# thodson-usgs/discontinuum

Measured on AMD Instinct MI355X. Metric: GP fits/sec (NLL+grad step) at n=8192 d=3, 1/2/4/8 MI355X, higher is better.
Workload: dtype f64

## Files before the change

### discontinuum_amd/_lib.py

```python
from __future__ import annotations

import ctypes as C
import os

_HERE = os.path.dirname(os.path.abspath(__file__))
LIB_PATH = os.path.join(_HERE, "libdgp_hip.so")

F64, F32 = 0, 1
MODEL_LOADEST, MODEL_RATING = 0, 1
OUT_NLL, OUT_QUAD, OUT_LOGDET, OUT_INFO, OUT_DTHETA, OUT_SUM_DR, OUT_DR_W0, OUT_SUM_DNOISE, OUT_LEN = 0, 1, 2, 3, 4, 28, 29, 31, 32
BUF_XT, BUF_A, BUF_T, BUF_S, BUF_Z, BUF_ALPHA = range(6)
BUF_SCAL = 7
OPT_LAUUM64_MAX_TILES, OPT_SYRK_SLOTS, OPT_TRTRI_SMALL, OPT_REFINE, OPT_SYRK_ORDER, OPT_LAUUM_ORDER, OPT_CHAIN_YIELD, OPT_FUSED_GRAD, OPT_GROUP_GEMM = range(9)
OPT_POTRF_SCHEDULE, OPT_POTRF_SWEEP, OPT_POTRF_SOLVE, OPT_POTRF_OVERLAP, OPT_POTRF_SLOTS, OPT_POTRF_TAIL, OPT_POTRF_TAIL_SWEEP = range(9, 16)
TIME_GRAM, TIME_POTRF, TIME_SYRK_SUM, TIME_SYRK_N, TIME_TRTRI, TIME_LAUUM, TIME_SOLVE, TIME_GRAD, TIME_SYRK_FLOP, TIME_COUNT = range(10)


class DGPLibraryError(RuntimeError):
    pass


class DGPError(RuntimeError):
    def __init__(self, code, where, msg):
        super().__init__(f"{where} failed with code {code}: {msg}")
        self.code = code


_vp, _i, _i64, _sz = C.c_void_p, C.c_int, C.c_int64, C.c_size_t
_dp = C.POINTER(C.c_double)

SIGNATURES = {
    "dgp_version": (_i, []),
    "dgp_last_error": (C.c_char_p, []),
    "dgp_model_ntheta": (_i, [_i, _i]),
    "dgp_composite_define": (_i, [C.POINTER(_i), _i, C.POINTER(_i)]),
    "dgp_padded_n": (_i64, [_i64]),
    "dgp_plan_create": (_i, [_i, _i, _i64, _i, C.POINTER(_vp)]),
# ... 93 lines not shown
```

### discontinuum_amd/csrc/dgp_api.hip

```cpp
#include <mutex>
#include <new>
#include <stdio.h>
#include <stdlib.h>
#include <string.h>
#include <utility>
#include <vector>

#include "../../include/dgp_hip.h"
#include "dgp_common.h"
#include "dgp_internal.h"

using namespace dgp;

static thread_local char g_err[256] = "";
static int fail(int code, const char* msg) {
  snprintf(g_err, sizeof(g_err), "%s", msg);
  return code;
}
static int hipfail(hipError_t e, const char* where) {
  snprintf(g_err, sizeof(g_err), "%s: %s", where, hipGetErrorString(e));
  return (int)e;
}

struct PinnedRing {
// ... 30 lines not shown
      if (have_ev[i]) (void)hipEventDestroy(ev[i]);
      if (buf[i]) (void)hipHostFree(buf[i]);
    }
  }
};

struct dgp_plan {
  int model, dtype, d, ntheta;
  PinnedRing ring;
  int* nsite_host;
  int B;
  size_t site_bytes;
  void* pre;
  void* pre2;
  int pre_ready;
  Tuning tune;
  int refine;
  int* nsite;
  const void* dr_w;
  int64_t n, N;
  size_t elem;
  char* ws;
  size_t ws_bytes;
  void *Xt, *A, *Tm, *S, *z, *alpha, *gpart, *spart, *scal, *snap;
  int* info;
  hipStream_t sc;
  int lookahead, early;
  int have_inputs, have_factor, have_inverse;
  hipStream_t s2, s3;
  hipEvent_t xev[8];
  int have_xev;
  hipEvent_t* ev;
  int nev;
  int timing, n_syrk, timed_valid;
  double syrk_flop;
  hipEvent_t* tev;
  hipEvent_t* sev;
  int nsev;
};
enum { TS_GRAM = 0, TS_POTRF, TS_TRTRI, TS_LAUUM, TS_SOLVE, TS_GRAD, TS_COUNT };

static size_t align_up(size_t x) { return (x + 255) & ~(size_t)255; }

struct Layout {
  size_t Xt, A, Tm, S, z, alpha, gpart, spart, scal, info, snap, total;
};
static Layout layout(const dgp_plan* p) {
  Layout L;
  const size_t e = p->elem, N = (size_t)p->N;
  size_t o = 0;
  L.Xt = o; o += align_up(e * N * p->d);
  L.A = o; o += align_up(e * N * N);
  L.Tm = o; o += align_up(e * N * N);
  L.S = o; o += align_up(e * N * N);
  L.z = o; o += align_up(e * N);
  L.alpha = o; o += align_up(e * N);
  L.gpart = o; o += align_up(e * (size_t)gram_grad_partials(p->N));
  L.spart = o; o += align_up(e * (size_t)solve_partials(p->N));
  L.scal = o; o += align_up(e * 16);
  L.info = o; o += align_up(sizeof(int) * POTRF_INFO_INTS);
  L.snap = o; o += align_up(e * 2 * DGP_TILE_HOST * DGP_TILE_HOST);
  L.total = o;
  return L;
}

static int default_lookahead() { return 2; }
static int group_size(int lookahead, int batch, long nbk) {
  if (!lookahead) return 0;
  if (const char* e = getenv("DGP_GROUP")) return atoi(e) < 2 ? 2 : atoi(e);
  if (batch >= 4) return 4;
  return nbk >= 256 ? 8 : (nbk >= 96 ? 4 : 2);
}

static int early_wg_cap() {
  const char* e = getenv("DGP_EARLY_WG_CAP");
  return e ? atoi(e) : 384;
}
#define EARLY_WG_CAP early_wg_cap()
static int early_reserved_cus() {
  const char* e = getenv("DGP_EARLY_RESERVED_CUS");
  const int v = e ? atoi(e) : 64;
  return v < 0 ? 0 : (v > 128 ? 128 : v);
}
#define EARLY_RESERVED_CUS early_reserved_cus()
// ... 98 lines not shown
  return 0;
}

int dgp_plan_set_workspace(dgp_plan* p, void* dev_ptr, size_t bytes) {
  if (!p || !dev_ptr) return fail(DGP_E_ARG, "dgp_plan_set_workspace: null");
  const Layout L = layout(p);
  if (bytes < dgp_plan_workspace_bytes(p))
    return fail(DGP_E_WORKSPACE, "dgp_plan_set_workspace: workspace too small");
  p->site_bytes = L.total;
  if (((uintptr_t)dev_ptr & 255) != 0) return fail(DGP_E_ARG, "dgp_plan_set_workspace: pointer must be 256-byte aligned");
  p->ws = (char*)dev_ptr;
  p->ws_bytes = bytes;
  p->Xt = p->ws + L.Xt;
  p->A = p->ws + L.A;
  p->Tm = p->ws + L.Tm;
  p->S = p->ws + L.S;
  p->z = p->ws + L.z;
  p->alpha = p->ws + L.alpha;
  p->gpart = p->ws + L.gpart;
  p->spart = p->ws + L.spart;
  p->scal = p->ws + L.scal;
  p->info = (int*)(p->ws + L.info);
  p->snap = p->ws + L.snap;
  p->pre = pre_scratch_bytes(p->B) ? (void*)(p->ws + L.total * (size_t)p->B) : nullptr;
  p->pre2 = p->pre ? (void*)((char*)p->pre + align_up(pre_scratch_bytes(p->B))) : nullptr;
  p->nsite = nullptr;
  p->dr_w = nullptr;
  if (p->B > 1) {
    p->nsite = (int*)(p->ws + L.total * (size_t)p->B + 2 * align_up(pre_scratch_bytes(p->B)));
    delete[] p->nsite_host;
    p->nsite_host = new (std::nothrow) int[(size_t)p->B];
    if (!p->nsite_host) return fail(DGP_E_ARG, "dgp_plan_set_workspace: out of host memory");
    for (int b = 0; b < p->B; ++b) p->nsite_host[b] = (int)p->n;
    hipError_t e = hipMemcpy(p->nsite, p->nsite_host, sizeof(int) * (size_t)p->B, hipMemcpyHostToDevice);
    if (e != hipSuccess) return hipfail(e, "dgp_plan_set_workspace: hipMemcpy");
  }
  p->have_inputs = p->have_factor = 0;
  return 0;
}

int dgp_plan_set_option(dgp_plan* p, int key, int64_t value) {
  if (!p) return fail(DGP_E_ARG, "dgp_plan_set_option: null plan");
  switch (key) {
    case DGP_OPT_LAUUM64_MAX_TILES:
      if (value < 0 || value > (1 << 30)) return fail(DGP_E_ARG, "dgp_plan_set_option: value out of range");
      p->tune.lauum64_max_tiles = (int)value;
// ... 19 lines not shown
      return 0;
    case DGP_OPT_GROUP_GEMM:
      p->tune.group_gemm = value ? 1 : 0;
      return 0;
    case DGP_OPT_POTRF_SCHEDULE:
      if (value < 0 || value > 1) return fail(DGP_E_ARG, "dgp_plan_set_option: value out of range");
      p->tune.potrf_schedule = (int)value;
      return 0;
    case DGP_OPT_POTRF_SWEEP:
    case DGP_OPT_POTRF_TAIL:
    case DGP_OPT_POTRF_TAIL_SWEEP:
      if (value < 0 || value > (1 << 20)) return fail(DGP_E_ARG, "dgp_plan_set_option: value out of range");
      (key == DGP_OPT_POTRF_SWEEP ? p->tune.potrf_sweep : key == DGP_OPT_POTRF_TAIL ? p->tune.potrf_tail : p->tune.potrf_tail_sweep) = (int)value;
      return 0;
    case DGP_OPT_POTRF_SOLVE:
      p->tune.potrf_solve = value ? 1 : 0;
      return 0;
    case DGP_OPT_POTRF_OVERLAP:
      p->tune.potrf_overlap = value ? 1 : 0;
      return 0;
    case DGP_OPT_POTRF_SLOTS:
      if (value < 1 || value > (1 << 20)) return fail(DGP_E_ARG, "dgp_plan_set_option: value out of range");
      p->tune.potrf_slots = (int)value;
      return 0;
    case DGP_OPT_REFINE:
      if (p->dtype != DGP_F32 && value) return fail(DGP_E_ARG, "dgp_plan_set_option: refinement applies to float32 plans");
      p->refine = value ? 1 : 0;
      return 0;
    default:
      return fail(DGP_E_ARG, "dgp_plan_set_option: unknown option");
  }
}
int dgp_plan_get_option(const dgp_plan* p, int key, int64_t* value) {
  if (!p || !value) return fail(DGP_E_ARG, "dgp_plan_get_option: null argument");
  switch (key) {
    case DGP_OPT_LAUUM64_MAX_TILES: *value = p->tune.lauum64_max_tiles; return 0;
    case DGP_OPT_SYRK_SLOTS: *value = p->tune.syrk_slots; return 0;
    case DGP_OPT_TRTRI_SMALL: *value = p->tune.trtri_small; return 0;
    case DGP_OPT_REFINE: *value = p->refine; return 0;
    case DGP_OPT_SYRK_ORDER: *value = p->tune.syrk_super; return 0;
    case DGP_OPT_LAUUM_ORDER: *value = p->tune.lauum_super; return 0;
    case DGP_OPT_CHAIN_YIELD: *value = p->tune.chain_yield; return 0;
    case DGP_OPT_FUSED_GRAD: *value = p->tune.fused_grad; return 0;
    case DGP_OPT_GROUP_GEMM: *value = p->tune.group_gemm; return 0;
    case DGP_OPT_POTRF_SCHEDULE:
      *value = p->tune.potrf_schedule < 0 ? (p->B >= 4 ? potrf_schedule_auto(p->B, p->N / DGP_TILE_HOST, p->elem) : 0) : p->tune.potrf_schedule;
      return 0;
    case DGP_OPT_POTRF_SWEEP: *value = p->tune.potrf_sweep; return 0;
    case DGP_OPT_POTRF_SOLVE: *value = p->tune.potrf_solve; return 0;
    case DGP_OPT_POTRF_OVERLAP: *value = p->tune.potrf_overlap; return 0;
    case DGP_OPT_POTRF_SLOTS: *value = p->tune.potrf_slots; return 0;
    case DGP_OPT_POTRF_TAIL: *value = p->tune.potrf_tail; return 0;
    case DGP_OPT_POTRF_TAIL_SWEEP: *value = p->tune.potrf_tail_sweep; return 0;
    default: return fail(DGP_E_ARG, "dgp_plan_get_option: unknown option");
  }
}

int dgp_plan_set_lookahead(dgp_plan* p, int level) {
  if (!p) return fail(DGP_E_ARG, "null plan");
  p->lookahead = level ? default_lookahead() : 0;
  p->early = level >= 2 && !getenv("DGP_NO_EARLY_TRTRI");
  return 0;
}

size_t dgp_plan_site_stride_bytes(const dgp_plan* p) { return p ? layout(p).total : 0; }

int dgp_plan_buffer(const dgp_plan* p, int which, void** dev_ptr, int64_t* ld) {
  if (!p || !dev_ptr || !p->ws) return fail(DGP_E_ARG, "dgp_plan_buffer: null / no workspace");
  void* q = nullptr;
  switch (which) {
    case DGP_BUF_XT: q = p->Xt; break;
    case DGP_BUF_A: q = p->A; break;
    case DGP_BUF_T: q = p->Tm; break;
    case DGP_BUF_S: q = p->S; break;
    case DGP_BUF_Z: q = p->z; break;
    case DGP_BUF_ALPHA: q = p->alpha; break;
// ... 273 lines not shown
  }
}

template <typename T>
static int run_grad(dgp_plan* p, const double* theta, void* dtheta, hipStream_t s) {
  return gram_grad<T>(p->model, p->d, (const T*)p->Xt, p->N, (int)p->n, theta, (const T*)p->S, (const T*)p->alpha,
                      (T*)p->gpart, (T*)dtheta, s, batch_of<T>(p), DGP_OUT_LEN, p->pre, p->pre_ready != 0);
}

template <typename T>
static int solve_overlap_mode(dgp_plan* p, hipStream_t s, hipStream_t* out) {
  static const int env = getenv("DGP_SOLVE_OVERLAP") ? atoi(getenv("DGP_SOLVE_OVERLAP")) : -1;
  const int mode = env >= 0 ? env : ((p->N >= 1024 && p->N <= 6144) ? 1 : 0);
  if (mode <= 0 || !p->lookahead || !p->ev || p->nev < 2) return 0;
  if (sizeof(T) == 4 && p->refine) return 0;
  if (mode == 1 && p->s2) {
    *out = p->s2;
    return 1;
  }
  StreamSet* st = stream_set(s);
  if (!st || make_stream(&st->rest, true)) return 0;
  *out = st->rest;
  return 2;
}

template <typename T>
static int fit_step(dgp_plan* p, const double* theta, const void* r, const void* noise, void* out, void* dr,
                    void* dnoise, int with_grad, hipStream_t s) {
  int rc;
  if ((rc = ensure_timing(p))) return rc;
  tick(p, TS_GRAM, 0, s);
  if ((rc = run_gram<T>(p, theta, noise, s))) return rc;
  tick(p, TS_GRAM, 1, s);
  if ((rc = ensure_async(p, s)) || (rc = ensure_early(p, s))) return rc;
  tick(p, TS_POTRF, 0, s);
  const int nbk = (int)(p->N / DGP_TILE_HOST);
  const bool early = early_applies(p) && p->s3 != nullptr;
  const Batch bt = batch_of<T>(p);
  if (early) {
    struct Early {
      dgp_plan* p;
      int ck[3];
      TrtriProgress st;
      int rc;
    } ctx{p, {nbk / 2, 3 * nbk / 4, 7 * nbk / 8}, {}, 0};
    if (const char* e = getenv("DGP_EARLY_CK")) {
// ... 17 lines not shown
      rc = potrf_split<T>((T*)p->A, p->N, (T*)p->Tm, (T*)p->scal, p->info, (T*)p->snap, s, p->sc, p->s2, p->ev,
                          p->timing ? p->sev : nullptr, &p->n_syrk, &p->syrk_flop, 3, ctx.ck, p->xev, on_ck, &ctx, split_start(p), group_size(p->lookahead, p->B, p->N / DGP_TILE_HOST), &p->tune);
    else
      rc = potrf<T>((T*)p->A, p->N, (T*)p->Tm, (T*)p->scal, p->info, group_size(p->lookahead, p->B, p->N / DGP_TILE_HOST), s, p->s2, p->ev,
                    p->timing ? p->sev : nullptr, &p->n_syrk, &p->syrk_flop, 3, ctx.ck, p->xev, on_ck, &ctx, bt);
    if (rc || (rc = ctx.rc)) return rc;
    tick(p, TS_POTRF, 1, s);
    tick(p, TS_TRTRI, 0, s);
    hipEventRecord(p->xev[3], s);
    hipStreamWaitEvent(p->s3, p->xev[3], 0);
    if ((rc = trtri_advance<T>((const T*)p->A, p->N, (T*)p->Tm, (T*)p->S, nbk, &ctx.st, p->s3, 0, nullptr, 0, 0, bt)))
      return rc;
    hipEventRecord(p->xev[4], p->s3);
    hipStreamWaitEvent(s, p->xev[4], 0);
    tick(p, TS_TRTRI, 1, s);
  } else {
    if ((rc = run_potrf<T>(p, s))) return rc;
    tick(p, TS_POTRF, 1, s);
    tick(p, TS_TRTRI, 0, s);
    if ((rc = run_trtri<T>(p, s))) return rc;
    tick(p, TS_TRTRI, 1, s);
  }
  const bool fused = with_grad && p->tune.fused_grad && lauum_grad_applies(p->model, p->N, bt);
  hipStream_t ss = s;
  const int ov = (with_grad && !fused) ? solve_overlap_mode<T>(p, s, &ss) : 0;
  if (ov) {
    hipEventRecord(p->ev[0], s);
    hipStreamWaitEvent(ss, p->ev[0], 0);
  }
  tick(p, TS_SOLVE, 0, ss);
  if ((rc = run_solve<T>(p, r, ss))) return rc;
  if ((rc = run_refine<T>(p, theta, r, noise, ss))) return rc;
  tick(p, TS_SOLVE, 1, ss);
  if (ov) hipEventRecord(p->ev[1], ss);
  p->timed_valid = 0;
  p->have_inverse = 0;
  if (!with_grad && ov) hipStreamWaitEvent(s, p->ev[1], 0);
  if (fused) {
    tick(p, TS_LAUUM, 0, s);
    void* staging = (p->pre && !p->pre_ready) ? p->ring.acquire(pre_scratch_bytes(p->B)) : nullptr;
    rc = lauum_grad<T>(p->model, p->d, (const T*)p->Tm, p->N, (T*)p->S, (const T*)p->Xt, (int)p->n, theta, (const T*)p->alpha,
                       (T*)p->gpart, (T*)out + DGP_OUT_DTHETA, s, bt, DGP_OUT_LEN, p->pre, p->pre_ready != 0, staging);
    if (staging) p->ring.commit(s);
    if (rc) return rc;
    p->pre_ready = 1;
    tick(p, TS_LAUUM, 1, s);
    tick(p, TS_GRAD, 0, s);
    tick(p, TS_GRAD, 1, s);
    p->timed_valid = p->timing && p->tev;
    p->have_inverse = 1;
  } else if (with_grad) {
    tick(p, TS_LAUUM, 0, s);
    if ((rc = run_lauum<T>(p, s))) return rc;
    tick(p, TS_LAUUM, 1, s);
    if (ov) hipStreamWaitEvent(s, p->ev[1], 0);
    tick(p, TS_GRAD, 0, s);
    if ((rc = run_grad<T>(p, theta, (T*)out + DGP_OUT_DTHETA, s))) return rc;
    tick(p, TS_GRAD, 1, s);
    p->timed_valid = p->timing && p->tev;
    p->have_inverse = 1;
  }
  const unsigned nwg = with_grad ? (unsigned)((p->n + 255) / 256) : 1u;
  finish_kernel<T><<<dim3(nwg, 1, (unsigned)bt.B), 256, 0, s>>>(
      (const T*)p->scal, p->info, (long)p->n, p->ntheta, !with_grad, (T*)out, bt.ws, bt.ws * (long)sizeof(T) / (long)sizeof(int), bt.ns,
      (const T*)p->alpha, (const T*)(with_grad ? p->dr_w : nullptr), (const T*)p->S, p->N, (T*)(with_grad ? dnoise : nullptr),
      (T*)(with_grad ? dr : nullptr), (T*)p->spart);
  p->have_factor = 1;
  return (int)hipGetLastError();
}

static size_t predict_site_bytes(const dgp_plan* p, int64_t m) {
  const size_t M = (size_t)round_up(m, DGP_TILE_HOST), e = p->elem;
  return align_up(e * M * p->d) + 2 * align_up(e * (size_t)p->N * M) + 3 * align_up(e * M) + align_up(e * 2 * PREDICT_SPLIT * M);
}
struct PreSlot {
  dgp_plan* p;
  void* staging;
  hipStream_t s;
  PreSlot(dgp_plan* plan, hipStream_t st) : p(plan), staging(plan->pre ? plan->ring.acquire(pre_scratch_bytes(plan->B)) : nullptr), s(st) {
    plan->pre_ready = 0;
  }
  ~PreSlot() {
    if (staging) p->ring.commit(s);
  }
};

template <typename T>
static int cross(dgp_plan* p, const double* theta, const void* Xs, int64_t m, void* work, void* Ks, hipStream_t s, long wbs = 0) {
  const long M = round_up(m, DGP_TILE_HOST);
  Batch wb;
  wb.B = p->B;
// ... 447 lines not shown
```

### discontinuum_amd/csrc/dgp_chol.hip

```cpp
#include <stdlib.h>
#include <string.h>
#include <algorithm>
#include <mutex>
#include "dgp_diag.h"
#include "dgp_gemm.h"
#include "dgp_gemm_dma.h"
#include "dgp_internal.h"
#include "dgp_schedule.h"

namespace dgp {

static constexpr int NB = DGP_TILE;
static constexpr int SMID_TABLE = 4096;
template <typename T>
struct Prefetch {
  static constexpr bool F64 = sizeof(T) == 8;
  static constexpr int LAUUM = F64 ? 2 : 4, TRTRI = F64 ? 1 : 4, SYRK = F64 ? 1 : 2;
};

#define DGP_INFO_CHAIN_TIMEOUT (-7)
#define CHAIN_WAIT_TICKS 200000000LL
__device__ __forceinline__ bool chain_reached(const int* word, int value) {
  return __hip_atomic_load(word, __ATOMIC_RELAXED, __HIP_MEMORY_SCOPE_AGENT) >= value;
}
// ... 105 lines not shown
    if (bi == bj && part == 1) return;
    syrk_tile<T, 64, 64, false, CMODE>(A, ld, k, nk, row0 + 64 * (part >> 1), col0 + 64 * (part & 1), smem);
  }
}

const Tuning& default_tuning() {
  static const Tuning t = [] {
    Tuning v;
    v.lauum64_max_tiles = getenv("DGP_LAUUM64") ? atoi(getenv("DGP_LAUUM64")) : 1000;
    v.syrk_slots = getenv("DGP_SYRK_SLOTS") ? atoi(getenv("DGP_SYRK_SLOTS")) : 512;
    v.trtri_small = getenv("DGP_TRTRI_SMALL") ? atol(getenv("DGP_TRTRI_SMALL")) : 1024;
    v.syrk_super = getenv("DGP_SYRK_ORDER") ? atoi(getenv("DGP_SYRK_ORDER")) : 0;
    v.lauum_super = getenv("DGP_LAUUM_ORDER") ? atoi(getenv("DGP_LAUUM_ORDER")) : 0;
    v.chain_yield = getenv("DGP_CHAIN_YIELD") ? atoi(getenv("DGP_CHAIN_YIELD")) : 1;
    v.fused_grad = getenv("DGP_FUSED_GRAD") ? atoi(getenv("DGP_FUSED_GRAD")) : 0;
    v.group_gemm = getenv("DGP_GROUP_GEMM") ? atoi(getenv("DGP_GROUP_GEMM")) : 0;
    v.potrf_schedule = getenv("DGP_POTRF_SCHEDULE") ? (atoi(getenv("DGP_POTRF_SCHEDULE")) != 0 ? 1 : 0) : -1;
    v.potrf_sweep = getenv("DGP_POTRF_SWEEP") ? std::max(0, atoi(getenv("DGP_POTRF_SWEEP"))) : 0;
    v.potrf_tail = getenv("DGP_POTRF_TAIL") ? std::max(0, atoi(getenv("DGP_POTRF_TAIL"))) : 0;
    v.potrf_tail_sweep = getenv("DGP_POTRF_TAIL_SWEEP") ? std::max(0, atoi(getenv("DGP_POTRF_TAIL_SWEEP"))) : 0;
    v.potrf_solve = getenv("DGP_POTRF_SOLVE") ? atoi(getenv("DGP_POTRF_SOLVE")) : 0;
    v.potrf_overlap = getenv("DGP_POTRF_OVERLAP") ? atoi(getenv("DGP_POTRF_OVERLAP")) : 0;
    v.potrf_slots = getenv("DGP_POTRF_SLOTS") ? std::max(1, atoi(getenv("DGP_POTRF_SLOTS"))) : 768;
    if (v.syrk_slots < 1) v.syrk_slots = 1;
    return v;
  }();
  return t;
}
int potrf_schedule_auto(int B, long nbk, int elem) { return (elem == 8 && B >= 32 && nbk > 4) ? 1 : 0; }
struct SyrkShape {
  int nfull, split;
  unsigned grid;
  explicit SyrkShape(int ntiles, int slots = 512) {
    if (slots < 1) slots = 1;
    const double cost[5] = {0, 1.0, 0.55, 0, 0.30};
    const int whole = ntiles / slots * slots, rem = ntiles - whole;
    nfull = ntiles;
    split = 1;
    double best = (ntiles + slots - 1) / slots * cost[1];
    for (int g = 2; g <= 4; g += 2) {
      const double c = whole / slots * cost[1] + (g * rem + slots - 1) / slots * cost[g];
      if (rem > 0 && c < best - 1e-9) {
        best = c;
        nfull = whole;
        split = g;
      }
// ... 808 lines not shown
    if (wcan > st->wdone[lvl]) st->wdone[lvl] = wcan;
    if (full > st->gdone[lvl]) st->gdone[lvl] = full;
  }
  if (early) st->pairs_used = nctr_pairs - el.pairs_left;
  return (int)hipGetLastError();
}

template <typename T>
static void trtri_group(const T* L, T* Tm, T* W, long N, int k0, int G, hipStream_t s, Batch bt) {
  for (int m = 1; m < G; m *= 2) {
    const int g0 = k0 / (2 * m), g1 = (k0 + G) / (2 * m);
    trtri_level<T, 0>(L, Tm, W, N, N, m, g0, g1, nullptr, s, bt);
    trtri_level<T, 1>(L, Tm, W, N, N, m, g0, g1, nullptr, s, bt);
  }
}

template <typename T>
int trtri(const T* L, const T* , long N, T* Tm, T* W, hipStream_t s, Batch bt,
          long ld) {
  TrtriProgress st;
  return trtri_advance<T>(L, N, Tm, W, (int)(N / NB), &st, s, 0, nullptr, 0, 0, bt, ld);
}

template <typename T>
__global__ __launch_bounds__(256, (TileCore<T, false, false>::OCC)) void lauum_kernel(const T* __restrict__ Tm, T* __restrict__ S, long ld,
                                                                                      int nbk, long bs, int super = 0) {
  Tm = site(Tm, bs);
  S = site(S, bs);
  using K = TileCore<T, false, false, 128, 128, Prefetch<T>::LAUUM, true, true>;
  using G = typename K::G;
  __shared__ T smem[K::SMEM_ELEMS];
  int bi, bj;
  if (super > 0) {
    const int x = (int)blockIdx.x & 7, j = (int)blockIdx.x >> 3, s2 = super * super;
    const int nsr = (nbk + super - 1) / super, st = (j / s2) * 8 + x;
    if (st >= nsr * (nsr + 1) / 2) return;
    int R, C;
    tri_decode(st, R, C);
    const int l = j % s2;
    bi = R * super + l / super;
    bj = C * super + l % super;
    if (bi >= nbk || bj > bi) return;
  } else {
    tri_decode(blockIdx.x, bi, bj);
  }
  typename G::acc_t acc[G::MI][G::NI];
  G::zero(acc);
  const T* base = Tm + (long)bi * NB * ld;
  T* out = S + (long)bi * NB * ld + (long)bj * NB;
  auto store = [&]() { K::foreach (acc, [&](int r, int c, T& v) { out[(long)r * ld + c] = v; }); };
  if (bi == bj) K::template run_tri<true, TRI_LOWER>(base + (long)bi * NB, ld, base + (long)bj * NB, ld, (nbk - bi) * (NB / 16), smem, acc, store);
  else K::template run_tri<true, TRI_ROW_LE>(base + (long)bi * NB, ld, base + (long)bj * NB, ld, (nbk - bi) * (NB / 16), smem, acc, store);
}

template <typename T>
__global__ __launch_bounds__(256, 2) void lauum64_kernel(const T* __restrict__ Tm, T* __restrict__ S, long ld, int nb64,
                                                         long bs) {
  Tm = site(Tm, bs);
  S = site(S, bs);
  using G = TileGemm<T, false, false, 64, 64>;
  __shared__ T smem[G::SMEM_ELEMS];
  int bi, bj;
  tri_decode(blockIdx.x, bi, bj);
  typename G::acc_t acc[G::MI][G::NI];
  G::zero(acc);
  const T* base = Tm + (long)bi * 64 * ld;
  G::template run<1, true>(base + (long)bi * 64, ld, base + (long)bj * 64, ld, (nb64 - bi) * (64 / 16), smem, acc);
  T* out = S + (long)bi * 64 * ld + (long)bj * 64;
  G::foreach (acc, [&](int r, int c, T& v) { out[(long)r * ld + c] = v; });
}

template <typename T>
int lauum(const T* Tm, long N, T* S, hipStream_t s, Batch bt) {
  const int nbk = (int)(N / NB);
  const int tiles = nbk * (nbk + 1) / 2;
  if ((long)tiles * bt.B <= bt.tuning().lauum64_max_tiles) {
    const int nb64 = 2 * nbk;
    lauum64_kernel<T><<<dim3((unsigned)(nb64 * (nb64 + 1) / 2), 1, (unsigned)bt.B), 256, 0, s>>>(Tm, S, N, nb64, bt.ws);
  } else {
    const int sup = bt.tuning().lauum_super;
    unsigned grid = (unsigned)tiles;
    if (sup > 0) {
      const int nsr = (nbk + sup - 1) / sup, nst = nsr * (nsr + 1) / 2;
      grid = (unsigned)((nst + 7) / 8 * 8 * sup * sup);
    }
    lauum_kernel<T><<<dim3(grid, 1, (unsigned)bt.B), 256, 0, s>>>(Tm, S, N, nbk, bt.ws, sup);
  }
  return (int)hipGetLastError();
}

template <typename T>
__global__ __launch_bounds__(256) void trmv_n_kernel(const T* __restrict__ Tm, long ld, const T* __restrict__ r, int n,
                                                     T* __restrict__ z, long bs, const int* __restrict__ ns, long rs) {
  Tm = site(Tm, bs);
  z = site(z, bs);
  r = site(r, rs);
  n = site_n(ns, n);
  const int lane = threadIdx.x & 63;
  const long i = (long)blockIdx.x * 4 + (threadIdx.x >> 6);
  const long jend = (i / NB + 1) * NB;
  const T* row = Tm + i * ld;
  T acc = T(0);
  for (long j = lane; j < jend; j += 64) acc += row[j] * (j < n ? r[j] : T(0));
  acc = wave_sum(acc);
  if (lane == 0) z[i] = acc;
}

#define DGP_TRMV_CHUNK 512
static inline int trmv_chunk(long N) { return N < 2048 ? 128 : DGP_TRMV_CHUNK; }
template <typename T>
// ... 297 lines not shown
  G::foreach (acc, [&](int r, int c, T& v) {
    const long q = (long)bq * NB + r, j = (long)bj * NB + c;
    if (q < ndraw && j < m) out[q * m + j] = v + (mean ? mean[j] : T(0));
  });
}

template <typename T>
int sample_draws(const T* L, long M, const T* Z, long Q, const T* mean, int m, int ndraw, T* out, hipStream_t s) {
  sample_draws_kernel<T><<<dim3((unsigned)(Q / NB), (unsigned)(M / NB)), 256, 0, s>>>(L, M, Z, Q, mean, m, ndraw, out);
  return (int)hipGetLastError();
}

#define DGP_INST(T)                                                                                              \
  template int posterior_cov<T>(const T*, long, long, T*, hipStream_t, int, long);                                          \
  template int sample_draws<T>(const T*, long, const T*, long, const T*, int, int, T*, hipStream_t);             \
  template int symv_lower<T>(const T*, long, const T*, int, const T*, T*, T*, T*, hipStream_t, Batch, long);     \
  template int potrf<T>(T*, long, T*, T*, int*, int, hipStream_t, hipStream_t, hipEvent_t*, hipEvent_t*, int*, double*, int, \
                        const int*, hipEvent_t*, void (*)(void*, int), void*, Batch, int, PotrfCarry*);                                                                                        \
  template int potrf_split<T>(T*, long, T*, T*, int*, T*, hipStream_t, hipStream_t, hipStream_t, hipEvent_t*, hipEvent_t*, int*, double*, \
                              int, const int*, hipEvent_t*, void (*)(void*, int), void*, int, int, const Tuning*);         \
  template int potrf_group<T>(T*, long, int, T*, T*, int*, int, int, hipStream_t);                                \
  template int trtri_advance<T>(const T*, long, T*, T*, int, TrtriProgress*, hipStream_t, int, int*, int, int, Batch, long);                   \
  template int trtri<T>(const T*, const T*, long, T*, T*, hipStream_t, Batch, long);                                        \
  template int lauum<T>(const T*, long, T*, hipStream_t, Batch);                                                      \
  template int solve<T>(const T*, long, const T*, int, T*, T*, T*, T*, hipStream_t, Batch);                           \
  template int refine_solve<T>(const T*, long, const T*, int, const double*, const T*, T*, T*, T*, T*, T*, hipStream_t, Batch, long, long); \
  template int finish<T>(const T*, const T*, long, int, T*, hipStream_t, Batch);                                      \
  template int predict_var<T>(const T*, long, const T*, long, T*, const T*, const T*, T*, T*, T*, hipStream_t, Batch, long);
DGP_INST(double)
DGP_INST(float)

}

#ifdef DGP_DIAG_LOG
extern "C" int dgp_debug_diag_log(unsigned long long* out_host) {
  return (int)hipMemcpyFromSymbol(out_host, HIP_SYMBOL(dgp::dgp_diag_log), sizeof(unsigned long long) * 4 * 1024);
}
#endif
```

### discontinuum_amd/csrc/dgp_internal.h

```cpp
#pragma once
#include <hip/hip_runtime.h>
#include <stdint.h>

#define DGP_TILE_HOST 128

namespace dgp {

inline long round_up(long n, long q) { return (n + q - 1) / q * q; }

#define DGP_MAX_BATCH_HOST 8
#define DGP_MAX_BATCH_SITES 1024
struct Tuning {
  int lauum64_max_tiles;
  int syrk_slots;
  long trtri_small;
  int syrk_super;
  int lauum_super;
  int chain_yield;
  int fused_grad;
  int group_gemm;
  int potrf_schedule;
  int potrf_sweep;
  int potrf_tail;
  int potrf_tail_sweep;
  int potrf_solve;
  int potrf_slots;
  int potrf_overlap;
};
const Tuning& default_tuning();
int potrf_schedule_auto(int B, long nbk, int elem);
struct Batch {
  int B = 1;
  long ws = 0;
  const int* ns = nullptr;
  const Tuning* tune = nullptr;
  void* W = nullptr;
  const Tuning& tuning() const { return tune ? *tune : default_tuning(); }
};
int model_ntheta(int model, int d);
int composite_define(const int* spec, int nspec);
bool composite_select(int model, int d);

template <typename T>
int pack_x(const T* X, int n, int d, long N, T* Xt, hipStream_t s, Batch bt = Batch());
template <typename T>
int gram_sym(int model, int d, const T* Xt, long N, int n, const double* theta, const T* noise, T* K, hipStream_t s,
             Batch bt = Batch(), void* pre_scratch = nullptr ,
             void* pre_staging = nullptr ,
             long k_stride = -1 , long noise_stride = -1 ,
             bool pre_ready = false );
// ... 44 lines not shown
                void* ck_ctx = nullptr, int k_start = 0 ,
                int G_old = 2 , const Tuning* tune = nullptr);
struct TrtriProgress {
  static constexpr int MAXLVL = 16;
  int wdone[MAXLVL] = {0}, gdone[MAXLVL] = {0};
  int pairs_used = 0;
};
template <typename T>
int trtri_advance(const T* L, long N, T* Tm, T* W, int ready_blocks, TrtriProgress* st, hipStream_t s, int wg_cap,
                  int* ctr , int nctr_pairs, int reserve_cus, Batch bt = Batch(),
                  long ld = 0 );
#define CHAIN_FLAG0 2
#define EARLY_CTR0 4
#define EARLY_CTR_PAIRS 125
#define POTRF_INFO_INTS (EARLY_CTR0 + 2 * EARLY_CTR_PAIRS + 4)
#define CHAIN_ABORT (POTRF_INFO_INTS - 4)
#define CHAIN_YIELD (POTRF_INFO_INTS - 3)
#define CHAIN_DIAG_DONE (POTRF_INFO_INTS - 2)
#define CHAIN_TICKET (POTRF_INFO_INTS - 1)
const unsigned char* reserved_cu_table(int nreserve, int* n_cu);
template <typename T>
int trtri(const T* L, const T* Dinv, long N, T* Tm, T* W, hipStream_t s, Batch bt = Batch(), long ld = 0);
template <typename T>
int lauum(const T* Tm, long N, T* S, hipStream_t s, Batch bt = Batch());
template <typename T>
int solve(const T* Tm, long N, const T* r, int n, T* z, T* alpha, T* partials, T* quad, hipStream_t s,
          Batch bt = Batch());
template <typename T>
int finish(const T* S, const T* alpha, long N, int n, T* dnoise, hipStream_t s, Batch bt = Batch());
template <typename T>
int refine_solve(const T* Tm, long N, const T* r, int n, const double* rho64, const T* rho32, T* z, T* delta, T* alpha,
                 T* partials, T* quad, hipStream_t s, Batch bt, long scratch_stride ,
                 long rho32_stride );
#define PREDICT_SPLIT 32
template <typename T>
int predict_var(const T* Tm, long N, const T* Ks, long M, T* V, const T* alpha, const T* kss, T* part, T* mean, T* var,
                hipStream_t s, Batch bt = Batch(), long wbs = 0);
long solve_partials(long N);
template <typename T>
int potrf_group(T* A, long ld, int nbk, T* Tinv, T* logdet, int* info, int k0, int W, hipStream_t s);
struct SlabMap {
  int W, world, rank;
  __host__ __device__ int gblock(int lb) const { return ((lb / W) * world + rank) * W + lb % W; }
};
template <typename T>
int gram_slab(int model, int d, const T* Xt, long N, int n, const double* theta, const T* noise, T* Aslab, long Cl,
              SlabMap sm, hipStream_t s);
// ... 29 lines not shown
```

### include/dgp_hip.h

```cpp
#ifndef DGP_HIP_H
#define DGP_HIP_H
#include <stddef.h>
#include <stdint.h>

#ifdef __cplusplus
extern "C" {
#endif

#define DGP_F64 0
#define DGP_F32 1
#define DGP_MODEL_LOADEST 0
#define DGP_MODEL_RATING 1

#define DGP_E_ARG (-1)
#define DGP_E_MODEL (-2)
#define DGP_E_WORKSPACE (-3)
#define DGP_E_STATE (-4)

#define DGP_OUT_NLL 0
#define DGP_OUT_QUAD 1
#define DGP_OUT_LOGDET 2
#define DGP_OUT_INFO 3
#define DGP_OUT_DTHETA 4
#define DGP_OUT_SUM_DR 28
// ... 23 lines not shown
size_t dgp_plan_workspace_bytes(const dgp_plan* plan);
int dgp_plan_set_batch(dgp_plan* plan, int batch);
int dgp_plan_batch(const dgp_plan* plan);
int dgp_plan_set_site_sizes(dgp_plan* plan, const int64_t* sizes_host, void* stream);
int dgp_plan_set_workspace(dgp_plan* plan, void* dev_ptr, size_t bytes);
int dgp_plan_set_dr_weights(dgp_plan* plan, const void* w_dev);
int dgp_plan_set_lookahead(dgp_plan* plan, int level);
#define DGP_OPT_LAUUM64_MAX_TILES 0
#define DGP_OPT_SYRK_SLOTS 1
#define DGP_OPT_TRTRI_SMALL 2
#define DGP_OPT_REFINE 3
#define DGP_OPT_SYRK_ORDER 4
#define DGP_OPT_LAUUM_ORDER 5
#define DGP_OPT_CHAIN_YIELD 6
#define DGP_OPT_FUSED_GRAD 7
#define DGP_OPT_GROUP_GEMM 8
#define DGP_OPT_POTRF_SCHEDULE 9
#define DGP_OPT_POTRF_SWEEP 10
#define DGP_OPT_POTRF_SOLVE 11
#define DGP_OPT_POTRF_OVERLAP 12
#define DGP_OPT_POTRF_SLOTS 13
#define DGP_OPT_POTRF_TAIL 14
#define DGP_OPT_POTRF_TAIL_SWEEP 15
int dgp_plan_set_option(dgp_plan* plan, int key, int64_t value);
int dgp_plan_get_option(const dgp_plan* plan, int key, int64_t* value_out);
int dgp_plan_buffer(const dgp_plan* plan, int which, void** dev_ptr, int64_t* ld);
size_t dgp_plan_site_stride_bytes(const dgp_plan* plan);

int dgp_set_inputs(dgp_plan* plan, const void* X_dev, void* stream);

int dgp_fit_step(dgp_plan* plan, const double* theta_host, const void* r_dev, const void* noise_dev,
                 void* out_dev, void* dr_dev, void* dnoise_dev, void* stream);

int dgp_factorize(dgp_plan* plan, const double* theta_host, const void* r_dev, const void* noise_dev,
                  void* out_dev, void* stream);

size_t dgp_predict_workspace_bytes(const dgp_plan* plan, int64_t m);
int dgp_predict(dgp_plan* plan, const double* theta_host, const void* Xs_dev, int64_t m, void* work_dev,
                size_t work_bytes, void* mean_dev, void* var_dev, void* stream);

int dgp_posterior_cov(dgp_plan* plan, const double* theta_host, const void* Xs_dev, int64_t m, void* work_dev,
                      size_t work_bytes, void* mean_dev, void* cov_dev, void* stream);

int dgp_sample_draws(int dtype, const void* L_dev, int64_t m, const void* Z_dev, int64_t ndraw, const void* mean_dev,
                     void* out_dev, void* stream);

// ... 83 lines not shown
```

Baseline: 118.0.

## Fuse alpha = S·r computation into LAUUM tile epilogue for f64

When the gradient path is taken without the fused-grad kernel and N is large, the LAUUM kernel computes per-tile partial products of the inverse S with the residual r while the tile is still hot. A new reduce kernel sums those partials into alpha and computes the quadratic term. This replaces the separate triangular solve stage and its overlap stream. It costs an extra N/128×N workspace buffer and extra shared-memory work in each LAUUM tile.

```diff
diff --git a/discontinuum_amd/_lib.py b/discontinuum_amd/_lib.py
--- a/discontinuum_amd/_lib.py
+++ b/discontinuum_amd/_lib.py
@@ -13,6 +13,7 @@
 BUF_SCAL = 7
 OPT_LAUUM64_MAX_TILES, OPT_SYRK_SLOTS, OPT_TRTRI_SMALL, OPT_REFINE, OPT_SYRK_ORDER, OPT_LAUUM_ORDER, OPT_CHAIN_YIELD, OPT_FUSED_GRAD, OPT_GROUP_GEMM = range(9)
 OPT_POTRF_SCHEDULE, OPT_POTRF_SWEEP, OPT_POTRF_SOLVE, OPT_POTRF_OVERLAP, OPT_POTRF_SLOTS, OPT_POTRF_TAIL, OPT_POTRF_TAIL_SWEEP = range(9, 16)
+OPT_ALPHA_EPILOGUE = 16
 TIME_GRAM, TIME_POTRF, TIME_SYRK_SUM, TIME_SYRK_N, TIME_TRTRI, TIME_LAUUM, TIME_SOLVE, TIME_GRAD, TIME_SYRK_FLOP, TIME_COUNT = range(10)
 
 
diff --git a/discontinuum_amd/csrc/dgp_api.hip b/discontinuum_amd/csrc/dgp_api.hip
--- a/discontinuum_amd/csrc/dgp_api.hip
+++ b/discontinuum_amd/csrc/dgp_api.hip
@@ -76,7 +76,7 @@
   size_t elem;
   char* ws;
   size_t ws_bytes;
-  void *Xt, *A, *Tm, *S, *z, *alpha, *gpart, *spart, *scal, *snap;
+  void *Xt, *A, *Tm, *S, *z, *alpha, *gpart, *spart, *scal, *snap, *apart;
   int* info;
   hipStream_t sc;
   int lookahead, early;
@@ -97,7 +97,7 @@
 static size_t align_up(size_t x) { return (x + 255) & ~(size_t)255; }
 
 struct Layout {
-  size_t Xt, A, Tm, S, z, alpha, gpart, spart, scal, info, snap, total;
+  size_t Xt, A, Tm, S, z, alpha, gpart, spart, scal, info, snap, apart, total;
 };
 static Layout layout(const dgp_plan* p) {
   Layout L;
@@ -114,6 +114,7 @@
   L.scal = o; o += align_up(e * 16);
   L.info = o; o += align_up(sizeof(int) * POTRF_INFO_INTS);
   L.snap = o; o += align_up(e * 2 * DGP_TILE_HOST * DGP_TILE_HOST);
+  L.apart = o; o += p->dtype == DGP_F64 ? align_up(e * (N / DGP_TILE_HOST) * N) : 0;
   L.total = o;
   return L;
 }
@@ -258,6 +259,7 @@
   p->scal = p->ws + L.scal;
   p->info = (int*)(p->ws + L.info);
   p->snap = p->ws + L.snap;
+  p->apart = p->dtype == DGP_F64 ? p->ws + L.apart : nullptr;
   p->pre = pre_scratch_bytes(p->B) ? (void*)(p->ws + L.total * (size_t)p->B) : nullptr;
   p->pre2 = p->pre ? (void*)((char*)p->pre + align_up(pre_scratch_bytes(p->B))) : nullptr;
   p->nsite = nullptr;
@@ -323,6 +325,10 @@
     case DGP_OPT_POTRF_SLOTS:
       if (value < 1 || value > (1 << 20)) return fail(DGP_E_ARG, "dgp_plan_set_option: value out of range");
       p->tune.potrf_slots = (int)value;
+      return 0;
+    case DGP_OPT_ALPHA_EPILOGUE:
+      if (value < -1 || value > 1) return fail(DGP_E_ARG, "dgp_plan_set_option: value out of range");
+      p->tune.alpha_epilogue = (int)value;
       return 0;
     case DGP_OPT_REFINE:
       if (p->dtype != DGP_F32 && value) return fail(DGP_E_ARG, "dgp_plan_set_option: refinement applies to float32 plans");
@@ -353,6 +359,7 @@
     case DGP_OPT_POTRF_SLOTS: *value = p->tune.potrf_slots; return 0;
     case DGP_OPT_POTRF_TAIL: *value = p->tune.potrf_tail; return 0;
     case DGP_OPT_POTRF_TAIL_SWEEP: *value = p->tune.potrf_tail_sweep; return 0;
+    case DGP_OPT_ALPHA_EPILOGUE: *value = p->tune.alpha_epilogue; return 0;
     default: return fail(DGP_E_ARG, "dgp_plan_get_option: unknown option");
   }
 }
@@ -672,6 +679,23 @@
   if (!st || make_stream(&st->rest, true)) return 0;
   *out = st->rest;
   return 2;
+}
+
+template <typename T>
+static bool alpha_epilogue_applies(const dgp_plan* p, const Batch& bt) {
+  if (sizeof(T) != 8 || !p->apart || p->tune.alpha_epilogue == 0 || !lauum_big_tiles(p->N, bt)) return false;
+  return p->tune.alpha_epilogue > 0 || p->N > 6144;
+}
+
+template <typename T>
+static int finish_step(dgp_plan* p, void* out, void* dr, void* dnoise, int with_grad, hipStream_t s, const Batch& bt) {
+  const unsigned nwg = with_grad ? (unsigned)((p->n + 255) / 256) : 1u;
+  finish_kernel<T><<<dim3(nwg, 1, (unsigned)bt.B), 256, 0, s>>>(
+      (const T*)p->scal, p->info, (long)p->n, p->ntheta, !with_grad, (T*)out, bt.ws, bt.ws * (long)sizeof(T) / (long)sizeof(int), bt.ns,
+      (const T*)p->alpha, (const T*)(with_grad ? p->dr_w : nullptr), (const T*)p->S, p->N, (T*)(with_grad ? dnoise : nullptr),
+      (T*)(with_grad ? dr : nullptr), (T*)p->spart);
+  p->have_factor = 1;
+  return (int)hipGetLastError();
 }
 
 template <typename T>
@@ -735,6 +759,27 @@
     tick(p, TS_TRTRI, 1, s);
   }
   const bool fused = with_grad && p->tune.fused_grad && lauum_grad_applies(p->model, p->N, bt);
+  if (with_grad && !fused && alpha_epilogue_applies<T>(p, bt)) {
+    p->timed_valid = 0;
+    p->have_inverse = 0;
+    if constexpr (sizeof(T) == 8) {
+      tick(p, TS_LAUUM, 0, s);
+      if ((rc = lauum<T>((const T*)p->Tm, p->N, (T*)p->S, s, bt, (const T*)r, (int)p->n, (T*)p->apart))) return rc;
+      tick(p, TS_LAUUM, 1, s);
+      tick(p, TS_SOLVE, 0, s);
+      const long ibs = bt.ws * (long)sizeof(T) / (long)sizeof(int);
+      if ((rc = alpha_reduce<T>((const T*)p->apart, p->N, (const T*)r, (int)p->n, (T*)p->alpha, (T*)p->scal + 1, (double*)p->spart, bt.ws,
+                                p->info + 1 , ibs, s, bt)))
+        return rc;
+      tick(p, TS_SOLVE, 1, s);
+    }
+    tick(p, TS_GRAD, 0, s);
+    if ((rc = run_grad<T>(p, theta, (T*)out + DGP_OUT_DTHETA, s))) return rc;
+    tick(p, TS_GRAD, 1, s);
+    p->timed_valid = p->timing && p->tev;
+    p->have_inverse = 1;
+    return finish_step<T>(p, out, dr, dnoise, with_grad, s, bt);
+  }
   hipStream_t ss = s;
   const int ov = (with_grad && !fused) ? solve_overlap_mode<T>(p, s, &ss) : 0;
   if (ov) {
@@ -773,13 +818,7 @@
     p->timed_valid = p->timing && p->tev;
     p->have_inverse = 1;
   }
-  const unsigned nwg = with_grad ? (unsigned)((p->n + 255) / 256) : 1u;
-  finish_kernel<T><<<dim3(nwg, 1, (unsigned)bt.B), 256, 0, s>>>(
-      (const T*)p->scal, p->info, (long)p->n, p->ntheta, !with_grad, (T*)out, bt.ws, bt.ws * (long)sizeof(T) / (long)sizeof(int), bt.ns,
-      (const T*)p->alpha, (const T*)(with_grad ? p->dr_w : nullptr), (const T*)p->S, p->N, (T*)(with_grad ? dnoise : nullptr),
-      (T*)(with_grad ? dr : nullptr), (T*)p->spart);
-  p->have_factor = 1;
-  return (int)hipGetLastError();
+  return finish_step<T>(p, out, dr, dnoise, with_grad, s, bt);
 }
 
 static size_t predict_site_bytes(const dgp_plan* p, int64_t m) {
diff --git a/discontinuum_amd/csrc/dgp_chol.hip b/discontinuum_amd/csrc/dgp_chol.hip
--- a/discontinuum_amd/csrc/dgp_chol.hip
+++ b/discontinuum_amd/csrc/dgp_chol.hip
@@ -151,6 +151,7 @@
     v.potrf_solve = getenv("DGP_POTRF_SOLVE") ? atoi(getenv("DGP_POTRF_SOLVE")) : 0;
     v.potrf_overlap = getenv("DGP_POTRF_OVERLAP") ? atoi(getenv("DGP_POTRF_OVERLAP")) : 0;
     v.potrf_slots = getenv("DGP_POTRF_SLOTS") ? std::max(1, atoi(getenv("DGP_POTRF_SLOTS"))) : 768;
+    v.alpha_epilogue = getenv("DGP_ALPHA_EPILOGUE") ? (atoi(getenv("DGP_ALPHA_EPILOGUE")) < 0 ? -1 : (atoi(getenv("DGP_ALPHA_EPILOGUE")) != 0 ? 1 : 0)) : -1;
     if (v.syrk_slots < 1) v.syrk_slots = 1;
     return v;
   }();
@@ -1005,9 +1006,12 @@
   return trtri_advance<T>(L, N, Tm, W, (int)(N / NB), &st, s, 0, nullptr, 0, 0, bt, ld);
 }
 
-template <typename T>
+template <typename T, bool ALPHA = false>
 __global__ __launch_bounds__(256, (TileCore<T, false, false>::OCC)) void lauum_kernel(const T* __restrict__ Tm, T* __restrict__ S, long ld,
-                                                                                      int nbk, long bs, int super = 0) {
+                                                                                      int nbk, long bs, int super = 0,
+                                                                                      const T* __restrict__ rv = nullptr, int n = 0,
+                                                                                      T* __restrict__ P = nullptr,
+                                                                                      const int* __restrict__ ns = nullptr) {
   Tm = site(Tm, bs);
   S = site(S, bs);
   using K = TileCore<T, false, false, 128, 128, Prefetch<T>::LAUUM, true, true>;
@@ -1034,6 +1038,115 @@
   auto store = [&]() { K::foreach (acc, [&](int r, int c, T& v) { out[(long)r * ld + c] = v; }); };
   if (bi == bj) K::template run_tri<true, TRI_LOWER>(base + (long)bi * NB, ld, base + (long)bj * NB, ld, (nbk - bi) * (NB / 16), smem, acc, store);
   else K::template run_tri<true, TRI_ROW_LE>(base + (long)bi * NB, ld, base + (long)bj * NB, ld, (nbk - bi) * (NB / 16), smem, acc, store);
+  if constexpr (ALPHA) {
+    constexpr int RP = NB + 1;
+    static_assert(2 * NB + 2 * 16 * RP <= K::SMEM_ELEMS, "the epilogue's strips do not fit the ring");
+    T* sri = smem;
+    T* srj = smem + NB;
+    T(*redr)[RP] = reinterpret_cast<T(*)[RP]>(smem + 2 * NB);
+    T(*redc)[RP] = reinterpret_cast<T(*)[RP]>(smem + 2 * NB + 16 * RP);
+    rv = site(rv, (long)n);
+    n = site_n(ns, n);
+    P = site(P, bs);
+    const int t = threadIdx.x;
+    {
+      const long g = (long)(t < NB ? bi : bj) * NB + (t & (NB - 1));
+      smem[t] = g < n ? rv[g] : T(0);
+    }
+    __threadfence();
+    __syncthreads();
+    const int ty = t >> 4, tx = t & 15;
+    const bool diag = bi == bj;
+    T ra[8], ca[8], rj[8];
+#pragma unroll
+    for (int b = 0; b < 8; ++b) ra[b] = ca[b] = T(0), rj[b] = srj[8 * tx + b];
+    const T* tile = S + (long)bi * NB * ld + (long)bj * NB + 8 * tx;
+#pragma unroll
+    for (int a = 0; a < 8; ++a) {
+      const int row = 8 * ty + a;
+      const T ri = sri[row];
+      T sv[8];
+      using V = typename Vec16<T>::type;
+      constexpr int VN = Vec16<T>::N;
+#pragma unroll
+      for (int q = 0; q < 8 / VN; ++q) {
+        const V v = *reinterpret_cast<const V*>(tile + (long)row * ld + q * VN);
+#pragma unroll
+        for (int e = 0; e < VN; ++e) sv[q * VN + e] = v[e];
+      }
+#pragma unroll
+      for (int b = 0; b < 8; ++b) {
+        const int col = 8 * tx + b;
+        const T vr = (diag && col > row) ? T(0) : sv[b];
+        const T vc = (diag && col >= row) ? T(0) : sv[b];
+        ra[a] += vr * rj[b];
+        ca[b] += vc * ri;
+      }
+    }
+#pragma unroll
+    for (int a = 0; a < 8; ++a) redr[tx][8 * ty + a] = ra[a], redc[ty][8 * tx + a] = ca[a];
+    __syncthreads();
+    const int e = t & (NB - 1);
+    if (t < NB) {
+      T sum = T(0);
+#pragma unroll
+      for (int x = 0; x < 16; ++x) sum += redr[x][e];
+      if (diag) {
+        T col = T(0);
+#pragma unroll
+        for (int y = 0; y < 16; ++y) col += redc[y][e];
+        sum += col;
+      }
+      P[(long)bj * ld + (long)bi * NB + e] = sum;
+    } else if (!diag) {
+      T sum = T(0);
+#pragma unroll
+      for (int y = 0; y < 16; ++y) sum += redc[y][e];
+      P[(long)bi * ld + (long)bj * NB + e] = sum;
+    }
+  }
+}
+
+template <typename T>
+__global__ __launch_bounds__(256) void alpha_reduce_kernel(const T* __restrict__ P, long N, int nbk, const T* __restrict__ rv, int n,
+                                                           T* __restrict__ alpha, long bs, T* __restrict__ quad,
+                                                           double* __restrict__ qpart, long qs, int* __restrict__ ticket, long ibs,
+                                                           const int* __restrict__ ns) {
+  P = site(P, bs);
+  rv = site(rv, (long)n);
+  n = site_n(ns, n);
+  alpha = site(alpha, bs);
+  quad = site(quad, bs);
+  qpart = site(qpart, qs);
+  ticket = site(ticket, ibs);
+  const int t = threadIdx.x, lane = t & 63, wv = t >> 6;
+  __shared__ double red[4];
+  __shared__ int last;
+  const long i = (long)blockIdx.x * 256 + t;
+  double q = 0.0;
+  if (i < N) {
+    T acc = T(0);
+#pragma unroll 8
+    for (int k = 0; k < nbk; ++k) acc += P[(long)k * N + i];
+    alpha[i] = acc;
+    if (i < n) q = (double)rv[i] * (double)acc;
+  }
+  q = wave_sum(q);
+  if (lane == 0) red[wv] = q;
+  __syncthreads();
+  if (t == 0) {
+    qpart[blockIdx.x] = red[0] + red[1] + red[2] + red[3];
+    __threadfence();
+    last = (gridDim.x == 1) || (atomicAdd(ticket, 1) == (int)gridDim.x - 1);
+  }
+  __syncthreads();
+  if (!last || t != 0) return;
+  __threadfence();
+  *ticket = 0;
+  double total = 0.0;
+  for (unsigned g = 0; g < gridDim.x; ++g) total += ((const volatile double*)qpart)[g];
+  quad[0] = (T)total;
+  if (sizeof(T) == 4) *reinterpret_cast<double*>(quad + 3) = total;
 }
 
 template <typename T>
@@ -1053,10 +1166,16 @@
   G::foreach (acc, [&](int r, int c, T& v) { out[(long)r * ld + c] = v; });
 }
 
-template <typename T>
-int lauum(const T* Tm, long N, T* S, hipStream_t s, Batch bt) {
+bool lauum_big_tiles(long N, const Batch& bt) {
+  const long nbk = N / NB;
+  return nbk * (nbk + 1) / 2 * bt.B > bt.tuning().lauum64_max_tiles;
+}
+
+template <typename T>
+int lauum(const T* Tm, long N, T* S, hipStream_t s, Batch bt, const T* r, int n, T* P) {
   const int nbk = (int)(N / NB);
   const int tiles = nbk * (nbk + 1) / 2;
+  if (r && (!P || !lauum_big_tiles(N, bt))) return -2;
   if ((long)tiles * bt.B <= bt.tuning().lauum64_max_tiles) {
     const int nb64 = 2 * nbk;
     lauum64_kernel<T><<<dim3((unsigned)(nb64 * (nb64 + 1) / 2), 1, (unsigned)bt.B), 256, 0, s>>>(Tm, S, N, nb64, bt.ws);
@@ -1067,8 +1186,21 @@
       const int nsr = (nbk + sup - 1) / sup, nst = nsr * (nsr + 1) / 2;
       grid = (unsigned)((nst + 7) / 8 * 8 * sup * sup);
     }
-    lauum_kernel<T><<<dim3(grid, 1, (unsigned)bt.B), 256, 0, s>>>(Tm, S, N, nbk, bt.ws, sup);
-  }
+    if (r) {
+      if constexpr (sizeof(T) == 8) lauum_kernel<T, true><<<dim3(grid, 1, (unsigned)bt.B), 256, 0, s>>>(Tm, S, N, nbk, bt.ws, sup, r, n, P, bt.ns);
+      else return -2;
+    } else {
+      lauum_kernel<T><<<dim3(grid, 1, (unsigned)bt.B), 256, 0, s>>>(Tm, S, N, nbk, bt.ws, sup);
+    }
+  }
+  return (int)hipGetLastError();
+}
+
+template <typename T>
+int alpha_reduce(const T* P, long N, const T* r, int n, T* alpha, T* quad, double* qpart, long qs, int* ticket, long ibs,
+                 hipStream_t s, Batch bt) {
+  alpha_reduce_kernel<T><<<dim3((unsigned)((N + 255) / 256), 1, (unsigned)bt.B), 256, 0, s>>>(P, N, (int)(N / NB), r, n, alpha, bt.ws, quad,
+                                                                                       qpart, qs, ticket, ibs, bt.ns);
   return (int)hipGetLastError();
 }
 
@@ -1412,7 +1544,8 @@
   template int potrf_group<T>(T*, long, int, T*, T*, int*, int, int, hipStream_t);                                \
   template int trtri_advance<T>(const T*, long, T*, T*, int, TrtriProgress*, hipStream_t, int, int*, int, int, Batch, long);                   \
   template int trtri<T>(const T*, const T*, long, T*, T*, hipStream_t, Batch, long);                                        \
-  template int lauum<T>(const T*, long, T*, hipStream_t, Batch);                                                      \
+  template int lauum<T>(const T*, long, T*, hipStream_t, Batch, const T*, int, T*);                                   \
+  template int alpha_reduce<T>(const T*, long, const T*, int, T*, T*, double*, long, int*, long, hipStream_t, Batch);  \
   template int solve<T>(const T*, long, const T*, int, T*, T*, T*, T*, hipStream_t, Batch);                           \
   template int refine_solve<T>(const T*, long, const T*, int, const double*, const T*, T*, T*, T*, T*, T*, hipStream_t, Batch, long, long); \
   template int finish<T>(const T*, const T*, long, int, T*, hipStream_t, Batch);                                      \
diff --git a/discontinuum_amd/csrc/dgp_internal.h b/discontinuum_amd/csrc/dgp_internal.h
--- a/discontinuum_amd/csrc/dgp_internal.h
+++ b/discontinuum_amd/csrc/dgp_internal.h
@@ -26,6 +26,7 @@
   int potrf_solve;
   int potrf_slots;
   int potrf_overlap;
+  int alpha_epilogue;
 };
 const Tuning& default_tuning();
 int potrf_schedule_auto(int B, long nbk, int elem);
@@ -116,7 +117,11 @@
 template <typename T>
 int trtri(const T* L, const T* Dinv, long N, T* Tm, T* W, hipStream_t s, Batch bt = Batch(), long ld = 0);
 template <typename T>
-int lauum(const T* Tm, long N, T* S, hipStream_t s, Batch bt = Batch());
+int lauum(const T* Tm, long N, T* S, hipStream_t s, Batch bt = Batch(), const T* r = nullptr, int n = 0, T* P = nullptr);
+bool lauum_big_tiles(long N, const Batch& bt);
+template <typename T>
+int alpha_reduce(const T* P, long N, const T* r, int n, T* alpha, T* quad, double* qpart, long qs, int* ticket, long ibs,
+                 hipStream_t s, Batch bt = Batch());
 template <typename T>
 int solve(const T* Tm, long N, const T* r, int n, T* z, T* alpha, T* partials, T* quad, hipStream_t s,
           Batch bt = Batch());
diff --git a/include/dgp_hip.h b/include/dgp_hip.h
--- a/include/dgp_hip.h
+++ b/include/dgp_hip.h
@@ -69,6 +69,7 @@
 #define DGP_OPT_POTRF_SLOTS 13
 #define DGP_OPT_POTRF_TAIL 14
 #define DGP_OPT_POTRF_TAIL_SWEEP 15
+#define DGP_OPT_ALPHA_EPILOGUE 16
 int dgp_plan_set_option(dgp_plan* plan, int key, int64_t value);
 int dgp_plan_get_option(const dgp_plan* plan, int key, int64_t* value_out);
 int dgp_plan_buffer(const dgp_plan* plan, int which, void** dev_ptr, int64_t* ld);
```

After: 119.2, median of 6. About the same (+1.0%).
